# lemma-osu/sknnr

Measured on NVIDIA B200. Metric: query-neighbors/sec (kneighbors+predict, k=7), higher is better.
Workload: dtype f16 operands / f32 accumulate filter + f64 refine

## Files before the change

### sknnr_b200/csrc/search_tc.cu

```cuda
#include <cstdio>
#include "common.cuh"
#include "kernels.h"
#include "tc_common.cuh"

#include <type_traits>

namespace sk {

template <int MT_, int NS_, int CAP_, int CAPE_> struct TcCfg {
    static constexpr int MT = MT_, NS = NS_, CAP = CAP_, CAPE = CAPE_;
    static constexpr int QT = MT * TC_M;
    static constexpr int EPI_WARPS = MT * 4 * NS;
    static constexpr int THREADS = (EPI_WARPS + MT + 1) * 32;
    static constexpr int LD = QT * NS;
    static constexpr int SORT = CAP <= 16 ? 16 : 32;
    static_assert(CAP <= SORT && CAP % 2 == 0, "candidate buffer shape");
    static constexpr int CH = 4 / NS;
};

__device__ unsigned long long g_tc_counters[8];

constexpr int TC_JOINT = 10;
constexpr int TC_JOINT_WIDE = 12;


template <int KC, int CAP, int LD, int NS, int J>
__device__ __forceinline__ ThrPr tc_compact(uint32_t bs0, uint32_t pub0, uint32_t c4, float thr, uint32_t pr) {
    static_assert(KC < CAP, "the buffer needs slack above KC");
    constexpr int SORT = CAP <= 16 ? 16 : 32;
    constexpr uint32_t IOFF = CAP * LD * 4, STEP = LD * 4;
    const uint32_t cs0 = bs0 + c4;
    const int cnt = (int)(pr / STEP);
    SK_CHECK((pr & (STEP - 1)) == c4 && cnt <= CAP);
    float s[SORT];
#pragma unroll
    for (int j = 0; j < SORT; ++j) s[j] = (j < CAP && j < cnt) ? lds_f32(cs0 + j * STEP) : SK_INF_F;
    sort_regs<SORT>(s);
    float t = s[KC - 1];
    if constexpr (NS == 2 && J < 2 * KC) {
        static_assert(LD == 512, "partner column = column ^ 256");
        const uint32_t mine = pub0 + c4, other = pub0 + (c4 ^ 1024u);
        float o[KC];
#pragma unroll
        for (int i = 0; i < KC; ++i) {
            st_shared_b32(mine + i * STEP, __float_as_uint(s[i]));
            o[i] = lds_f32(other + i * STEP);
        }
        const float joint = tc_union_rank<KC, J, SORT>(s, o);
        t = fminf(t, joint);
    }
    t = fminf(t, thr);
    uint32_t w = cs0;
#pragma unroll 4
    for (int j = 0; j < CAP; ++j) {
        const float v = lds_f32(cs0 + j * STEP);
        const int id = lds_s32(cs0 + IOFF + j * STEP);
        if (j < cnt && v < t) {
            st_shared_b32(w, __float_as_uint(v));
            st_shared_b32(w + IOFF, (uint32_t)id);
            w += STEP;
        }
    }
    ThrPr out;
    out.thr = t;
    out.pr = w - bs0;
    return out;
}

template <int KC, int CAP, int LD, int CAPE, int NS, int J, bool DBG>
__device__ __noinline__ ThrPr tc_drain(uint32_t bs0, uint32_t pqv0, uint32_t pqi0, uint32_t pub0, uint32_t c4,
                                       float thr, uint32_t pr, uint32_t pqo, int dbg) {
    constexpr uint32_t IOFF = CAP * LD * 4, STEP = LD * 4, ES = LD * 32;
    constexpr uint32_t FULL = (CAP - 2) * STEP, LAST = (CAP - 1) * STEP;
    const int n_me = (int)(pqo / ES);
    SK_CHECK((pqo & (ES - 1)) == 8u * c4 && n_me <= CAPE);
    const int n_it = __reduce_max_sync(SK_FULL, n_me);
    for (int it = 0; it < n_it; ++it) {
        const bool act = it < n_me;
        if (__any_sync(SK_FULL, act && pr >= FULL)) {
            if (DBG && (dbg & 8) && (threadIdx.x & 31) == 0) atomicAdd(&g_tc_counters[4], 1ull);
            const ThrPr c = tc_compact<KC, CAP, LD, NS, J>(bs0, pub0, c4, thr, pr);
            thr = c.thr;
// ... 20 lines not shown
    out.thr = thr;
    out.pr = pr;
    out.n_it = n_it;
    return out;
}

template <int LD, int CAPE, bool DBG>
__device__ __forceinline__ void tc_chunk(const uint32_t (&r)[32], int idb, uint32_t pqv0, uint32_t pqi0, float &thr,
                                         uint32_t &pqo, int dbg) {
    constexpr uint32_t ES = LD * 32, PQ_END = CAPE * ES;
    float v[32];
#pragma unroll
    for (int i = 0; i < 32; ++i) v[i] = __uint_as_float(r[i]);
    float g[4];
#pragma unroll
    for (int o = 0; o < 4; ++o) {
        const float *w = v + 8 * o;
        g[o] = fminf(fminf(fminf(fminf(w[0], w[1]), w[2]), fminf(fminf(w[3], w[4]), w[5])), fminf(w[6], w[7]));
    }
    const float m = fminf(fminf(fminf(g[0], g[1]), g[2]), g[3]);
    const bool hit = m < thr;
    if constexpr (DBG) {
        const unsigned hits = __ballot_sync(SK_FULL, hit);
        if ((dbg & 8) && (threadIdx.x & 31) == 0) {
            atomicAdd(&g_tc_counters[0], 1ull);
            if (hits) atomicAdd(&g_tc_counters[1], 1ull);
        }
        if (hits == 0u) return;
        if (dbg & 1) return;
    } else {
        if (!__any_sync(SK_FULL, hit)) return;
    }
    unsigned ov[4];
#pragma unroll
    for (int o = 0; o < 4; ++o) ov[o] = __ballot_sync(SK_FULL, g[o] < thr);
#pragma unroll
    for (int o = 0; o < 4; ++o) {
        if (ov[o] == 0u) continue;
        const bool p = g[o] < thr;
        const bool room = pqo < PQ_END;
        SK_CHECK(pqo < PQ_END + ES);
        tc_dump8(p && room, pqv0 + pqo, pqi0 + (pqo >> 3), v + 8 * o, idb + 8 * o);
        if (p && !room) thr = fminf(thr, g[o]);
        if (p && room) pqo += ES;
        if (DBG && (dbg & 8) && p) atomicAdd(&g_tc_counters[room ? 2 : 5], 1ull);
    }
}

template <int CH, class F>
__device__ __forceinline__ void tc_epi_job(uint32_t (&R)[CH][32], uint32_t tcol, uint32_t afull_addr,
                                           uint32_t parity, uint32_t aempty_addr, int lane, F &&proc) {
    mbar_wait_addr(afull_addr, parity);
    tc_fence_after();
    if constexpr (CH == 2) {
        tmem_ld64_issue(tcol, R[0], R[1]);
    } else if constexpr (CH == 4) {
        tmem_ld64_issue(tcol, R[0], R[1]);
        tmem_ld64_issue(tcol + 64, R[2], R[3]);
    } else {
        uint32_t dep = 0;
#pragma unroll
        for (int c = 0; c < CH; ++c) tmem_ld32_issue(tcol + 32 * c, R[c], dep);
    }
#pragma unroll
    for (int c = 0; c < CH; ++c) tmem_ld_wait(R[c]);
    tc_fence_before();
    __syncwarp();
    if (lane == 0) mbar_arrive_addr(aempty_addr);
    if constexpr (CH >= 1) proc(R[0], std::integral_constant<int, 0>{});
    if constexpr (CH >= 2) proc(R[1], std::integral_constant<int, 1>{});
    if constexpr (CH >= 3) proc(R[2], std::integral_constant<int, 2>{});
    if constexpr (CH >= 4) proc(R[3], std::integral_constant<int, 3>{});
}

template <int KC, int MT, int NS, int CAP, int CAPE, int J, bool DBG>
__global__ void __launch_bounds__(TcCfg<MT, NS, CAP, CAPE>::THREADS, 1)
search_tc_kernel(const __half *__restrict__ qimg, const __half *__restrict__ rimg, int kc_tot,
                 int n_rtiles, int nstage, int n_seed, int seed_stride, long long n_q,
                 int *__restrict__ cand_idx, float *__restrict__ cand_thr, int dbg,
                 const float *__restrict__ init_thr, const int *__restrict__ n_rows_dev) {
    using Cfg = TcCfg<MT, NS, CAP, CAPE>;
    if (n_rows_dev) {
        const long long n_dev = *n_rows_dev;
        if ((long long)blockIdx.x * Cfg::QT >= n_dev) return;
        n_q = min(n_q, n_dev);
    }
    constexpr int LD = Cfg::LD, EPI_WARPS = Cfg::EPI_WARPS;
    constexpr bool JOINT = NS == 2 && J < 2 * KC;
    constexpr int KCP = JOINT ? KC : 0;
    extern __shared__ __align__(128) unsigned char smem_raw[];
    const uint32_t a_bytes = (uint32_t)kc_tot * TC_M * TC_ROWB;
    const uint32_t b_bytes = (uint32_t)kc_tot * TC_N * TC_ROWB;
    unsigned char *Qs = smem_raw;
    unsigned char *Rs = Qs + MT * a_bytes;
    float *buf_s = reinterpret_cast<float *>(Rs + (size_t)nstage * b_bytes);
    int *buf_i = reinterpret_cast<int *>(buf_s + CAP * LD);
    float *pq_v = reinterpret_cast<float *>(buf_i + CAP * LD);
    int *pq_i = reinterpret_cast<int *>(pq_v + CAPE * LD * 8);
    float *pub = reinterpret_cast<float *>(pq_i + CAPE * LD);
    uint64_t *full = reinterpret_cast<uint64_t *>(pub + KCP * LD);
    uint64_t *empty = full + nstage;
    uint64_t *afull = empty + nstage;
    uint64_t *aempty = afull + TC_SLOTS;
    uint64_t *qbar = aempty + TC_SLOTS;
    uint32_t *tmem_slot = reinterpret_cast<uint32_t *>(qbar + 1);

    const int warp = __shfl_sync(SK_FULL, (int)(threadIdx.x >> 5), 0), lane = threadIdx.x & 31;
    if (threadIdx.x == 0) {
        for (int s = 0; s < nstage; ++s) {
            mbar_init(&full[s], 1);
            mbar_init(&empty[s], MT);
        }
        for (int a = 0; a < TC_SLOTS; ++a) {
            mbar_init(&afull[a], 1);
            mbar_init(&aempty[a], 4 * NS);
        }
        mbar_init(qbar, 1);
        fence_mbar_init();
    }
    if (warp == EPI_WARPS) tmem_alloc(tmem_slot, 512);
    tc_fence_before();
    __syncthreads();
    tc_fence_after();
    const uint32_t tmem_base = *tmem_slot;
    const long long qtile = blockIdx.x;
    const int ksteps = kc_tot >> 1;
    const int n_seq = n_seed + n_rtiles;

    if (warp == EPI_WARPS + MT) {
        if (lane == 0) {
            mbar_expect_tx(qbar, MT * a_bytes);
            bulk_g2s(Qs, (const unsigned char *)qimg + (size_t)qtile * MT * a_bytes, MT * a_bytes, qbar);
            int sn = 0;
            uint32_t wrap_par = 1;
            bool wrapped = false;
            const unsigned char *rbase = (const unsigned char *)rimg;
            for (int tn = 0; tn < n_seq; ++tn) {
                if (wrapped) mbar_wait(&empty[sn], wrap_par);
                const int tile = tn < n_seed ? tn * seed_stride : tn - n_seed;
                if (DBG && (dbg & 4) && wrapped) {
                    mbar_arrive(&full[sn]);
                } else {
                    mbar_expect_tx(&full[sn], b_bytes);
                    bulk_g2s(Rs + (size_t)sn * b_bytes, rbase + (size_t)tile * b_bytes, b_bytes, &full[sn]);
                }
                if (++sn == nstage) {
                    sn = 0;
                    wrap_par = wrapped ? (wrap_par ^ 1u) : 0u;
                    wrapped = true;
                }
            }
        }
        __syncwarp();
    } else if (warp >= EPI_WARPS) {
        const int h = warp - EPI_WARPS;
        mbar_wait(qbar, 0);
        const uint32_t a_lbo = TC_M * TC_ROWB, b_lbo = TC_N * TC_ROWB;
        const uint64_t desc_hi = (uint64_t)((128u >> 4) | (1u << 14)) << 32;
        const uint32_t a_lo0 = (((smem_u32(Qs) + h * a_bytes) >> 4) & 0x3fffu) | (((a_lbo >> 4) & 0x3fffu) << 16);
        const uint32_t b_lo0 = ((smem_u32(Rs) >> 4) & 0x3fffu) | (((b_lbo >> 4) & 0x3fffu) << 16);
        const uint32_t a_kstep = (2 * a_lbo) >> 4, b_kstep = (2 * b_lbo) >> 4;
        const uint32_t b_img = b_bytes >> 4;
        int s = 0;
        uint32_t full_par = 0, b_lo_s = b_lo0;
        for (int t = 0; t < n_seq; ++t) {
            const int j = t * MT + h;
            const uint32_t sl = (uint32_t)j & (TC_SLOTS - 1);
            mbar_wait(&full[s], full_par);
            if (j >= TC_SLOTS) mbar_wait(&aempty[sl], (uint32_t)(((j >> 2) - 1) & 1));
            tc_fence_after();
            const uint32_t d_tmem = tmem_base + sl * TC_N;
            SK_CHECK(s >= 0 && s < nstage && sl < TC_SLOTS);
            if (elect_one()) {
                if (DBG && (dbg & 16)) {
                    uint32_t a2 = a_lo0, b2 = b_lo_s;
                    tc_mma_f16(d_tmem, desc_hi | a2, desc_hi | b2, TC_IDESC, 0u);
                    for (int ks = 1; ks < ksteps; ++ks) {
                        a2 += a_kstep;
                        b2 += b_kstep;
                        tc_mma_f16(d_tmem, desc_hi | a2, desc_hi | b2, TC_IDESC, 1u);
                    }
                }
                uint32_t a_lo = a_lo0, b_lo = b_lo_s;
                tc_mma_f16(d_tmem, desc_hi | a_lo, desc_hi | b_lo, TC_IDESC, 0u);
#pragma unroll 4
                for (int ks = 1; ks < ksteps; ++ks) {
                    a_lo += a_kstep;
                    b_lo += b_kstep;
                    tc_mma_f16(d_tmem, desc_hi | a_lo, desc_hi | b_lo, TC_IDESC, 1u);
                }
                tc_commit(&afull[sl]);
                tc_commit(&empty[s]);
            }
            __syncwarp();
            b_lo_s += b_img;
            if (++s == nstage) {
                s = 0;
                full_par ^= 1u;
                b_lo_s = b_lo0;
            }
        }
    } else {
        constexpr int CH = Cfg::CH;
        const int col = threadIdx.x;
        const int p = warp / (MT * 4);
        const int h = (warp >> 2) % MT;
        const int qslot = h * TC_M + (warp & 3) * 32 + lane;
        const uint32_t tlane = tmem_base + (((uint32_t)((warp & 3) * 32)) << 16) + (uint32_t)(p * CH * 32);
        float thr = SK_INF_F;
        if (init_thr) {
            const long long q_me = qtile * Cfg::QT + qslot;
            thr = q_me < n_q ? init_thr[q_me] : -SK_INF_F;
        }
        uint32_t R[CH][32];
        int t = 0;
        const uint32_t afull_a0 = smem_u32(afull), aempty_a0 = smem_u32(aempty);

        const uint32_t bs0 = smem_u32(smem_raw) + MT * a_bytes + (uint32_t)nstage * b_bytes;
        const uint32_t pqv0 = bs0 + 2u * CAP * LD * 4u, pqi0 = pqv0 + (uint32_t)CAPE * LD * 32u;
        const uint32_t pub0 = pqi0 + (uint32_t)CAPE * LD * 4u;
        const uint32_t c4 = 4u * (uint32_t)col;
        if constexpr (KCP > 0) {
#pragma unroll
            for (int i = 0; i < KCP; ++i) st_shared_b32(pub0 + c4 + i * (LD * 4), __float_as_uint(SK_INF_F));
        }

        if (n_seed > 0) {
            static_assert(2 * CAP >= TC_GROUPS, "group minima are parked in the candidate buffers");
            float *gcol = buf_s + col;
#pragma unroll
            for (int g = 0; g < TC_GROUPS; ++g) gcol[g * LD] = SK_INF_F;
            const bool fine = n_seed * CH < TC_GROUPS;
            for (; t < n_seed; ++t) {
                const int j = t * MT + h, sl = j & (TC_SLOTS - 1);
                const int g0 = (t * CH) & (TC_GROUPS - 1);
                tc_epi_job<CH>(R, tlane + (uint32_t)(sl * TC_N), afull_a0 + 8u * sl, (uint32_t)((j >> 2) & 1),
                               aempty_a0 + 8u * sl, lane,
                               [&](const uint32_t (&r)[32], auto ic) {
                                   constexpr int c = decltype(ic)::value;
                                   if (!fine) {
                                       float *g = gcol + (g0 + c) * LD;
                                       *g = fminf(*g, tc_min32(r));
                                   } else {
#pragma unroll
                                       for (int o = 0; o < 4; ++o) {
                                           float m = __uint_as_float(r[8 * o]);
#pragma unroll
                                           for (int e = 1; e < 8; ++e) m = fminf(m, __uint_as_float(r[8 * o + e]));
                                           float *g = gcol + (((t * CH + c) * 4 + o) & (TC_GROUPS - 1)) * LD;
                                           *g = fminf(*g, m);
                                       }
                                   }
                               });
            }
            float gm[TC_GROUPS];
#pragma unroll
            for (int g = 0; g < TC_GROUPS; ++g) gm[g] = gcol[g * LD];
            sort_regs<TC_GROUPS>(gm);
            thr = gm[KC - 1];
            if constexpr (KCP > 0) {
#pragma unroll
                for (int i = 0; i < KC; ++i) st_shared_b32(pub0 + c4 + i * (LD * 4), __float_as_uint(gm[i]));
                asm volatile("bar.sync %0, 64;" ::"r"(1 + (warp & (MT * 4 - 1))) : "memory");
                float o[KC];
#pragma unroll
                for (int i = 0; i < KC; ++i) o[i] = lds_f32(pub0 + (c4 ^ 1024u) + i * (LD * 4));
                const float joint = tc_union_rank<KC, J, TC_GROUPS>(gm, o);
                thr = fminf(thr, joint);
            }
        }

        constexpr uint32_t ES = LD * 32;
        uint32_t pr = c4;
        uint32_t pqo = 8u * c4;
        int since_drain = 1;
        const int early_tiles = max(64, n_rtiles >> 3);
        for (; t < n_seq; ++t) {
            const int j = t * MT + h, sl = j & (TC_SLOTS - 1);
            const int idb = (t - n_seed) * TC_N + p * CH * 32;
            tc_epi_job<CH>(R, tlane + (uint32_t)(sl * TC_N), afull_a0 + 8u * sl, (uint32_t)((j >> 2) & 1),
                           aempty_a0 + 8u * sl, lane,
                           [&](const uint32_t (&r)[32], auto ic) {
                               constexpr int c = decltype(ic)::value;
                               tc_chunk<LD, CAPE, DBG>(r, idb + c * 32, pqv0, pqi0, thr, pqo, dbg);
                           });
            constexpr int DRAIN_EVERY = 8;
            bool now;
            if constexpr (CAPE >= 4 && NS == 2) {
                now = (((t - n_seed) & (DRAIN_EVERY - 1)) == DRAIN_EVERY - 1) | (--since_drain == 0);
                if ((t - n_seed) < early_tiles) now |= __any_sync(SK_FULL, pqo >= (uint32_t)(CAPE - 1) * ES);
            } else {
                now = __any_sync(SK_FULL, pqo >= ES);
            }
            if (now) {
                if (DBG && (dbg & 8) && lane == 0) atomicAdd(&g_tc_counters[3], 1ull);
                if (DBG && (dbg & 32)) {
                    pqo = 8u * c4;
                    since_drain = -1;
                    continue;
                }
                const ThrPr d = tc_drain<KC, CAP, LD, CAPE, NS, J, DBG>(bs0, pqv0, pqi0, pub0, c4, thr, pr, pqo, dbg);
                thr = d.thr;
                pr = d.pr;
                pqo = 8u * c4;
                since_drain = d.n_it >= CAPE - 1 ? 1 : (d.n_it >= CAPE - 2 ? 2 : -1);
            }
        }

        {
            const ThrPr d = tc_drain<KC, CAP, LD, CAPE, NS, J, DBG>(bs0, pqv0, pqi0, pub0, c4, thr, pr, pqo, dbg);
            const ThrPr c = tc_compact<KC, CAP, LD, NS, J>(bs0, pub0, c4, d.thr, d.pr);
            thr = c.thr;
            pr = c.pr;
        }
        const int cnt = (int)(pr / (uint32_t)(LD * 4));
        SK_CHECK(cnt < KC && cnt <= 16 / NS);
        const long long q = qtile * Cfg::QT + qslot;
        if (q < n_q) {
            constexpr int KOUT = 16 / NS;
            int4 *dst = reinterpret_cast<int4 *>(cand_idx + (q * NS + p) * KOUT);
#pragma unroll
            for (int jj = 0; jj < KOUT; jj += 4) {
                int4 v;
                v.x = (jj + 0 < cnt) ? buf_i[(jj + 0) * LD + col] : -1;
                v.y = (jj + 1 < cnt) ? buf_i[(jj + 1) * LD + col] : -1;
                v.z = (jj + 2 < cnt) ? buf_i[(jj + 2) * LD + col] : -1;
                v.w = (jj + 3 < cnt) ? buf_i[(jj + 3) * LD + col] : -1;
                dst[jj / 4] = v;
            }
            cand_thr[q * NS + p] = thr;
        }
    }

    tc_fence_before();
    __syncthreads();
    tc_fence_after();
    if (warp == EPI_WARPS) tmem_dealloc(tmem_base, 512);
    if (DBG && (dbg & 8) && blockIdx.x == gridDim.x - 1 && threadIdx.x == 0)
        printf("tc counters (up to the last CTA): chunks %llu events %llu queued %llu drains %llu compactions %llu dropped %llu\n",
               g_tc_counters[0], g_tc_counters[1], g_tc_counters[2], g_tc_counters[3], g_tc_counters[4],
               g_tc_counters[5]);
}

int g_tc_debug = 0;

static constexpr int TC_MT = 2;

size_t search_tc_smem_bytes(int kc_tot, int nstage, int ns, int cape) {
    const size_t a = (size_t)kc_tot * TC_M * TC_ROWB, b = (size_t)kc_tot * TC_N * TC_ROWB;
    const size_t ld = (size_t)TC_MT * TC_M * ns, cap = ns == 2 ? 16 : 32, kcp = (ns == 2 && kc_tot <= 6) ? 8 : 0;
    return TC_MT * a + nstage * b + ld * 4 * (2 * cap + (size_t)cape * 9 + kcp) +
           (size_t)(2 * nstage + 2 * TC_SLOTS + 1) * 8 + 16;
}

int search_tc_pick_config(int kc_tot) {
    const int capes[2] = {4, 2};
    for (int ci = 0; ci < 2; ++ci)
        for (int s = 4; s >= 2; --s)
            if (search_tc_smem_bytes(kc_tot, s, 2, capes[ci]) <= 227 * 1024 &&
                search_tc_smem_bytes(kc_tot, s, 1, capes[ci]) <= 227 * 1024)
                return s | (capes[ci] << 8);
    return 0;
}

int search_tc_seed_stride(int n_rtiles, int seed_stride) {
    if (seed_stride <= 0) seed_stride = 4;
    if (n_rtiles < 64) return 1;
    if (n_rtiles < 192) return seed_stride < 2 ? seed_stride : 2;
    return seed_stride;
}
int search_tc_seed_tiles(int n_rtiles, int seed_stride) {
    const int st = search_tc_seed_stride(n_rtiles, seed_stride);
    return (n_rtiles + st - 1) / st;
}

template <int KC, int MT, int NS, int CAP, int CAPE, int J, bool DBG>
static cudaError_t launch_tc_dbg(const __half *qimg, const __half *rimg, int kc_tot, int n_rtiles, int nstage,
                                 int seed_stride, long long n_q, int *cand_idx, float *cand_thr,
                                 const float *init_thr, const int *n_rows_dev, cudaStream_t st) {
    using Cfg = TcCfg<MT, NS, CAP, CAPE>;
    const size_t smem = search_tc_smem_bytes(kc_tot, nstage, NS, CAPE);
    cudaError_t e = cudaFuncSetAttribute(search_tc_kernel<KC, MT, NS, CAP, CAPE, J, DBG>,
                                         cudaFuncAttributeMaxDynamicSharedMemorySize, 227 * 1024);
    if (e != cudaSuccess) return e;
    const long long n_qtiles = (n_q + Cfg::QT - 1) / Cfg::QT;
    const int n_seed = init_thr ? 0 : search_tc_seed_tiles(n_rtiles, seed_stride);
    search_tc_kernel<KC, MT, NS, CAP, CAPE, J, DBG><<<(unsigned)n_qtiles, Cfg::THREADS, smem, st>>>(
        qimg, rimg, kc_tot, n_rtiles, nstage, n_seed, search_tc_seed_stride(n_rtiles, seed_stride), n_q, cand_idx,
        cand_thr, g_tc_debug, init_thr, n_rows_dev);
    return cudaGetLastError();
}

template <int KC, int MT, int NS, int CAP>
static cudaError_t launch_tc(const __half *qimg, const __half *rimg, int kc_tot, int n_rtiles, int nstage,
                             int cape, int seed_stride, int wide_joint, long long n_q, int *cand_idx, float *cand_thr,
                             const float *init_thr, const int *n_rows_dev, cudaStream_t st) {
    constexpr int JLO = NS == 2 ? TC_JOINT : 1, JMID = NS == 2 ? TC_JOINT_WIDE : 1, JHI = NS == 2 ? 2 * KC : 1;
    const bool deep = kc_tot > 6;
#define SK_TC_GO(CAPE_, J_, DBG_)                                                                                  \
    return launch_tc_dbg<KC, MT, NS, CAP, CAPE_, J_, DBG_>(qimg, rimg, kc_tot, n_rtiles, nstage, seed_stride, n_q, \
                                                           cand_idx, cand_thr, init_thr, n_rows_dev, st)
    if (g_tc_debug && cape == 4 && !deep) SK_TC_GO(4, JLO, true);
    if (cape == 4 && !deep && NS == 2 && wide_joint) SK_TC_GO(4, JMID, false);
    if (cape == 4 && !deep) SK_TC_GO(4, JLO, false);
    if (cape == 4) SK_TC_GO(4, JHI, false);
    if (cape == 2) SK_TC_GO(2, JHI, false);
#undef SK_TC_GO
    return cudaErrorInvalidValue;
}

cudaError_t launch_search_tc(const __half *qimg, const __half *rimg, int kc_tot, int n_rtiles,
                             long long n_q, int ns, int config, int seed_stride, int wide_joint, int *cand_idx,
                             float *cand_thr, const float *init_thr, const int *n_rows_dev, cudaStream_t st) {
    if (n_q <= 0) return cudaSuccess;
    const int nstage = config & 0xff, cape = (config >> 8) & 0xff;
    if (ns == 2)
        return launch_tc<8, TC_MT, 2, 16>(qimg, rimg, kc_tot, n_rtiles, nstage, cape, seed_stride, wide_joint, n_q,
                                          cand_idx, cand_thr, init_thr, n_rows_dev, st);
    if (ns == 1)
        return launch_tc<16, TC_MT, 1, 32>(qimg, rimg, kc_tot, n_rtiles, nstage, cape, seed_stride, 0, n_q,
                                           cand_idx, cand_thr, init_thr, n_rows_dev, st);
    return cudaErrorInvalidValue;
}

}
```

### sknnr_b200/csrc/refine.cu

```cuda
#include "common.cuh"
#include "kernels.h"

namespace sk {

constexpr int REFINE_WARPS = 8;

__device__ __forceinline__ double dist2_lane(const double *__restrict__ zq, const double *__restrict__ r,
                                             int d, int h) {
    double acc = 0.0;
    for (int k = h; k < d; k += 16) {
        const double df = zq[k] - __ldg(r + k);
        acc = __fma_rn(df, df, acc);
    }
    return acc;
}
template <int DJ>
__device__ __forceinline__ double dist2_lane_regs(const double (&zr)[DJ], const double *__restrict__ r, int d,
                                                  int h) {
    double rv[DJ];
#pragma unroll
    for (int j = 0; j < DJ; ++j) rv[j] = (h + 16 * j < d) ? __ldg(r + h + 16 * j) : 0.0;
    double acc = 0.0;
#pragma unroll
    for (int j = 0; j < DJ; ++j) {
// ... 45 lines not shown
    return __double2float_ru(t);
}

template <int DJ>
__global__ void __launch_bounds__(REFINE_WARPS * 32)
refine_kernel(RefineArgs a, FinishParams fp) {
    const int warp = __shfl_sync(SK_FULL, (int)(threadIdx.x >> 5), 0), lane = threadIdx.x & 31;
    const long long q = (long long)blockIdx.x * REFINE_WARPS + warp;
    if (q >= a.n_q || (a.n_rows_dev && q >= *a.n_rows_dev)) return;
    if (a.n_rows_dev && *a.n_rows_dev < a.bypass_rows) {
        if (lane == 0) a.fb_list[atomicAdd(a.fb_count, 1)] = a.row_map ? a.row_map[q] : (int)q;
        return;
    }
    const double *zq = a.z64 + q * a.d;

    const int half = lane >> 4, hl = lane & 15;
    const bool small = a.kc <= 16;
    int id = 0x7fffffff;
    double d2 = SK_INF_D;
    const int my_c = lane < a.kc ? a.cand_idx[q * a.kc + lane] : -1;
    double zr[DJ > 0 ? DJ : 1];
    if constexpr (DJ > 0) {
#pragma unroll
        for (int j = 0; j < DJ; ++j) zr[j] = (hl + 16 * j < a.d) ? zq[hl + 16 * j] : 0.0;
    }
#pragma unroll 4
    for (int i = 0; 2 * i < a.kc; ++i) {
        const int c = __shfl_sync(SK_FULL, my_c, (2 * i + half) & 31);
        const bool have = c >= 0 && c < a.n_ref;
        double acc = 0.0;
        if (have) {
            if constexpr (DJ > 0)
                acc = dist2_lane_regs<DJ>(zr, a.ref64 + (long long)c * a.d, a.d, hl);
            else
                acc = dist2_lane(zq, a.ref64 + (long long)c * a.d, a.d, hl);
        }
        acc = dist2_reduce16(acc);
        if (small) {
            const double other = __shfl_xor_sync(SK_FULL, acc, 16);
            if ((lane >> 1) == i && lane < 16 && my_c >= 0 && my_c < a.n_ref) {
                id = my_c;
                d2 = (lane & 1) == half ? acc : other;
            }
        } else if (have && hl == (i & 15)) {
            id = c;
            d2 = acc;
        }
    }
    double qn = 0.0;
    for (int k = lane; k < a.d; k += 32) {
        const double df = zq[k] - a.mu[k];
        qn += df * df;
    }
#pragma unroll
    for (int o = 16; o > 0; o >>= 1) qn += __shfl_xor_sync(SK_FULL, qn, o);

    if (small)
        warp_sort_pairs<double, 16>(d2, id, lane);
    else
        warp_sort_pairs<double, 32>(d2, id, lane);

    const int kk = fp.k + (fp.exclude_self ? 1 : 0);
    const double kth = __shfl_sync(SK_FULL, d2, kk - 1);
    float thr = a.cand_thr[q * a.n_thr];
    for (int i = 1; i < a.n_thr; ++i) thr = fminf(thr, a.cand_thr[q * a.n_thr + i]);
    bool ok;
    if (thr == SK_INF_F) {
        ok = true;
    } else {
        const double bound = (double)thr * a.thr_scale + qn - a.eps_s * (qn + a.r2max);
        ok = kth < bound && qn < a.qn_limit;
    }
    if (!ok) {
        if (lane == 0) {
            const int pos = atomicAdd(a.fb_count, 1);
            a.fb_list[pos] = a.row_map ? a.row_map[q] : (int)q;
            if (a.fb_thr) a.fb_thr[pos] = retry_threshold(kth, qn, a);
        }
        return;
    }
    finish_query(fp, q, sqrt_padded(d2), id, lane);
}

template <int DJ>
__global__ void __launch_bounds__(REFINE_WARPS * 32)
refine2_kernel(RefineArgs a, FinishParams fp) {
    const int warp = __shfl_sync(SK_FULL, (int)(threadIdx.x >> 5), 0), lane = threadIdx.x & 31;
    const int seg = lane >> 4, hl = lane & 15;
    const long long n_rows = a.n_rows_dev ? min((long long)*a.n_rows_dev, a.n_q) : a.n_q;
    const long long q0 = ((long long)blockIdx.x * REFINE_WARPS + warp) * 2;
    if (q0 >= n_rows) return;
    const bool live = q0 + seg < n_rows;
    const long long q = live ? q0 + seg : q0;
    if (a.n_rows_dev && n_rows < a.bypass_rows) {
        if (live && hl == 0) a.fb_list[atomicAdd(a.fb_count, 1)] = a.row_map ? a.row_map[q] : (int)q;
        return;
    }
    const double *zq = a.z64 + q * a.d;
    double zr[DJ];
#pragma unroll
    for (int j = 0; j < DJ; ++j) zr[j] = (hl + 16 * j < a.d) ? zq[hl + 16 * j] : 0.0;
    const int my_c = hl < a.kc ? a.cand_idx[q * a.kc + hl] : -1;
    int id = 0x7fffffff;
    double d2 = SK_INF_D;
    auto take = [&](int i) {
        const int c = __shfl_sync(SK_FULL, my_c, i, 16);
        SK_CHECK(c >= -1 && c < a.n_ref);
        const bool have = c >= 0 && c < a.n_ref;
        double acc = 0.0;
        if (have) acc = dist2_lane_regs<DJ>(zr, a.ref64 + (long long)c * a.d, a.d, hl);
        acc = dist2_reduce16(acc);
        if (have && hl == i) {
            id = c;
            d2 = acc;
        }
    };
    const unsigned vm = __ballot_sync(SK_FULL, my_c >= 0);
    int n_step = 8;
    if (a.kc == 16) {
        int worst = 0;
        bool prefix = true;
#pragma unroll
        for (int hlf = 0; hlf < 4; ++hlf) {
            const unsigned m = (vm >> (8 * hlf)) & 0xffu;
            const int n = __popc(m);
            prefix = prefix && (m == ((1u << n) - 1u));
            worst = max(worst, n);
        }
        if (prefix) n_step = worst;
        for (int i = 0; i < n_step; ++i) {
            take(i);
            take(8 + i);
        }
    } else {
#pragma unroll 4
        for (int i = 0; i < a.kc; ++i) take(i);
    }
    double qn = 0.0;
    for (int k = hl; k < a.d; k += 16) {
        const double df = zq[k] - a.mu[k];
        qn += df * df;
    }
#pragma unroll
    for (int o = 8; o > 0; o >>= 1) qn += __shfl_xor_sync(SK_FULL, qn, o);
    warp_sort_pairs<double, 16>(d2, id, hl);

    const int kk = fp.k + (fp.exclude_self ? 1 : 0);
    const double kth = __shfl_sync(SK_FULL, d2, kk - 1, 16);
    float thr = a.cand_thr[q * a.n_thr];
    for (int i = 1; i < a.n_thr; ++i) thr = fminf(thr, a.cand_thr[q * a.n_thr + i]);
    bool ok = true;
    if (thr != SK_INF_F) ok = kth < (double)thr * a.thr_scale + qn - a.eps_s * (qn + a.r2max) && qn < a.qn_limit;
    if (live && !ok && hl == 0) {
        const int pos = atomicAdd(a.fb_count, 1);
        a.fb_list[pos] = a.row_map ? a.row_map[q] : (int)q;
        if (a.fb_thr) a.fb_thr[pos] = retry_threshold(kth, qn, a);
    }
    finish_query_w<16>(fp, q, sqrt_padded(d2), id, hl, live && ok);
}

cudaError_t launch_refine(const RefineArgs &a, const FinishParams &fp, cudaStream_t st) {
    if (a.n_q <= 0) return cudaSuccess;
    if (a.kc <= 16 && a.d <= 64) {
        const long long grid2 = (a.n_q + 2 * REFINE_WARPS - 1) / (2 * REFINE_WARPS);
        switch ((a.d + 15) / 16) {
            case 1: refine2_kernel<1><<<(unsigned)grid2, REFINE_WARPS * 32, 0, st>>>(a, fp); break;
            case 2: refine2_kernel<2><<<(unsigned)grid2, REFINE_WARPS * 32, 0, st>>>(a, fp); break;
            case 3: refine2_kernel<3><<<(unsigned)grid2, REFINE_WARPS * 32, 0, st>>>(a, fp); break;
            default: refine2_kernel<4><<<(unsigned)grid2, REFINE_WARPS * 32, 0, st>>>(a, fp); break;
        }
        return cudaGetLastError();
    }
    const long long grid = (a.n_q + REFINE_WARPS - 1) / REFINE_WARPS;
    switch (a.d <= 64 ? (a.d + 15) / 16 : 0) {
        case 1: refine_kernel<1><<<(unsigned)grid, REFINE_WARPS * 32, 0, st>>>(a, fp); break;
        case 2: refine_kernel<2><<<(unsigned)grid, REFINE_WARPS * 32, 0, st>>>(a, fp); break;
        case 3: refine_kernel<3><<<(unsigned)grid, REFINE_WARPS * 32, 0, st>>>(a, fp); break;
        case 4: refine_kernel<4><<<(unsigned)grid, REFINE_WARPS * 32, 0, st>>>(a, fp); break;
        default: refine_kernel<0><<<(unsigned)grid, REFINE_WARPS * 32, 0, st>>>(a, fp); break;
    }
    return cudaGetLastError();
}

constexpr int EXACT_THREADS = 256;

__device__ __forceinline__ double exact_pair(const ExactArgs &a, long long q, int j) {
    if (a.metric == 0) {
        const double *zq = a.z64 + q * a.d;
        const double *r = a.ref64 + (long long)j * a.d;
        return dist2_serial(zq, r, a.d);
    }
    const uint16_t *qc = a.qcodes + q * a.ldq;
    const uint16_t *rc = a.rcodes + (long long)j * a.n_trees;
    double num = 0.0;
    for (int t = 0; t < a.n_trees; ++t) {
        if (qc[t] != rc[t]) num = __dadd_rn(num, a.w[t]);
    }
    return num / a.wsum;
}

__device__ void finish_query_block(const FinishParams &p, long long q, double *sd, int *si, double *key,
                                   long long *sec, int kk) {
    __shared__ double sh_denom;
    __shared__ int sh_zero;
    const long long row = p.row_offset + q;
    if (threadIdx.x == 0) {
        if (p.exclude_self) {
            int pos = 0;
            for (int c = 0; c < kk; ++c)
                if ((long long)si[c] == row) { pos = c; break; }
            for (int c = pos; c + 1 < kk; ++c) {
                sd[c] = sd[c + 1];
                si[c] = si[c + 1];
            }
        }
        if (p.deterministic) {
            const double scale = fmax(sd[p.k - 1], 1.0);
            for (int c = 0; c < p.k; ++c) {
                key[c] = rint((sd[c] / scale) * p.round_scale) / p.round_scale;
                long long diff = (long long)si[c] - row;
                if (diff < 0) diff = -diff;
                sec[c] = (diff << 31) | (long long)si[c];
            }
            for (int c = 1; c < p.k; ++c) {
// ... 181 lines not shown
```

Before: 120.6 million.

## Make tensor-core search kernel persistent over query tiles with Q-tile reuse barrier

Turns the search kernel into a grid-stride persistent kernel capped at four blocks per SM. Each block loops over query tiles and reuses its barriers, TMEM slots and stage ring across tiles, with a new qfree barrier guarding reloads of the query image. The next query tile is also prefetched into L2. This removes per-block launch, setup and TMEM allocation costs and lets the reference stream continue across tiles. In exchange it adds cross-tile barrier parity bookkeeping and a serial dependence on the Q buffer, and the kernel declares one block per SM, so the 4x grid only runs as extra waves.

After: 120.4 million (median of 6 runs). No clear change (-0.2%).

```diff
diff --git a/sknnr_b200/csrc/search_tc.cu b/sknnr_b200/csrc/search_tc.cu
--- a/sknnr_b200/csrc/search_tc.cu
+++ b/sknnr_b200/csrc/search_tc.cu
@@ -1,3 +1,4 @@
+#include <algorithm>
 #include <cstdio>
 #include "common.cuh"
 #include "kernels.h"
@@ -184,9 +185,10 @@
     using Cfg = TcCfg<MT, NS, CAP, CAPE>;
     if (n_rows_dev) {
         const long long n_dev = *n_rows_dev;
-        if ((long long)blockIdx.x * Cfg::QT >= n_dev) return;
         n_q = min(n_q, n_dev);
     }
+    const long long n_qtiles = (n_q + Cfg::QT - 1) / Cfg::QT;
+    if ((long long)blockIdx.x >= n_qtiles) return;
     constexpr int LD = Cfg::LD, EPI_WARPS = Cfg::EPI_WARPS;
     constexpr bool JOINT = NS == 2 && J < 2 * KC;
     constexpr int KCP = JOINT ? KC : 0;
@@ -205,7 +207,8 @@
     uint64_t *afull = empty + nstage;
     uint64_t *aempty = afull + TC_SLOTS;
     uint64_t *qbar = aempty + TC_SLOTS;
-    uint32_t *tmem_slot = reinterpret_cast<uint32_t *>(qbar + 1);
+    uint64_t *qfree = qbar + 1;
+    uint32_t *tmem_slot = reinterpret_cast<uint32_t *>(qfree + 1);
 
     const int warp = __shfl_sync(SK_FULL, (int)(threadIdx.x >> 5), 0), lane = threadIdx.x & 31;
     if (threadIdx.x == 0) {
@@ -218,6 +221,7 @@
             mbar_init(&aempty[a], 4 * NS);
         }
         mbar_init(qbar, 1);
+        mbar_init(qfree, MT);
         fence_mbar_init();
     }
     if (warp == EPI_WARPS) tmem_alloc(tmem_slot, 512);
@@ -225,38 +229,45 @@
     __syncthreads();
     tc_fence_after();
     const uint32_t tmem_base = *tmem_slot;
-    const long long qtile = blockIdx.x;
     const int ksteps = kc_tot >> 1;
-    const int n_seq = n_seed + n_rtiles;
+    const int n_seq = (DBG && (dbg & 64)) ? n_seed : n_seed + n_rtiles;
 
     if (warp == EPI_WARPS + MT) {
         if (lane == 0) {
-            mbar_expect_tx(qbar, MT * a_bytes);
-            bulk_g2s(Qs, (const unsigned char *)qimg + (size_t)qtile * MT * a_bytes, MT * a_bytes, qbar);
             int sn = 0;
             uint32_t wrap_par = 1;
             bool wrapped = false;
-            const unsigned char *rbase = (const unsigned char *)rimg;
-            for (int tn = 0; tn < n_seq; ++tn) {
-                if (wrapped) mbar_wait(&empty[sn], wrap_par);
-                const int tile = tn < n_seed ? tn * seed_stride : tn - n_seed;
-                if (DBG && (dbg & 4) && wrapped) {
-                    mbar_arrive(&full[sn]);
-                } else {
-                    mbar_expect_tx(&full[sn], b_bytes);
-                    bulk_g2s(Rs + (size_t)sn * b_bytes, rbase + (size_t)tile * b_bytes, b_bytes, &full[sn]);
-                }
-                if (++sn == nstage) {
-                    sn = 0;
-                    wrap_par = wrapped ? (wrap_par ^ 1u) : 0u;
-                    wrapped = true;
+            const unsigned char *rbase = (const unsigned char *)rimg, *qbase = (const unsigned char *)qimg;
+            int it = 0;
+            for (long long qtile = blockIdx.x; qtile < n_qtiles; qtile += gridDim.x, ++it) {
+                if (it > 0) mbar_wait(qfree, (uint32_t)((it - 1) & 1));
+                mbar_expect_tx(qbar, MT * a_bytes);
+                bulk_g2s(Qs, qbase + (size_t)qtile * MT * a_bytes, MT * a_bytes, qbar);
+                if (qtile + gridDim.x < n_qtiles)
+                    asm volatile("cp.async.bulk.prefetch.L2.global [%0], %1;" ::"l"(
+                                     qbase + (size_t)(qtile + gridDim.x) * MT * a_bytes),
+                                 "r"(MT * a_bytes)
+                                 : "memory");
+                for (int tn = 0; tn < n_seq; ++tn) {
+                    if (wrapped) mbar_wait(&empty[sn], wrap_par);
+                    const int tile = tn < n_seed ? tn * seed_stride : tn - n_seed;
+                    if (DBG && (dbg & 4) && wrapped) {
+                        mbar_arrive(&full[sn]);
+                    } else {
+                        mbar_expect_tx(&full[sn], b_bytes);
+                        bulk_g2s(Rs + (size_t)sn * b_bytes, rbase + (size_t)tile * b_bytes, b_bytes, &full[sn]);
+                    }
+                    if (++sn == nstage) {
+                        sn = 0;
+                        wrap_par = wrapped ? (wrap_par ^ 1u) : 0u;
+                        wrapped = true;
+                    }
                 }
             }
         }
         __syncwarp();
     } else if (warp >= EPI_WARPS) {
         const int h = warp - EPI_WARPS;
-        mbar_wait(qbar, 0);
         const uint32_t a_lbo = TC_M * TC_ROWB, b_lbo = TC_N * TC_ROWB;
         const uint64_t desc_hi = (uint64_t)((128u >> 4) | (1u << 14)) << 32;
         const uint32_t a_lo0 = (((smem_u32(Qs) + h * a_bytes) >> 4) & 0x3fffu) | (((a_lbo >> 4) & 0x3fffu) << 16);
@@ -265,42 +276,49 @@
         const uint32_t b_img = b_bytes >> 4;
         int s = 0;
         uint32_t full_par = 0, b_lo_s = b_lo0;
-        for (int t = 0; t < n_seq; ++t) {
-            const int j = t * MT + h;
-            const uint32_t sl = (uint32_t)j & (TC_SLOTS - 1);
-            mbar_wait(&full[s], full_par);
-            if (j >= TC_SLOTS) mbar_wait(&aempty[sl], (uint32_t)(((j >> 2) - 1) & 1));
-            tc_fence_after();
-            const uint32_t d_tmem = tmem_base + sl * TC_N;
-            SK_CHECK(s >= 0 && s < nstage && sl < TC_SLOTS);
-            if (elect_one()) {
-                if (DBG && (dbg & 16)) {
-                    uint32_t a2 = a_lo0, b2 = b_lo_s;
-                    tc_mma_f16(d_tmem, desc_hi | a2, desc_hi | b2, TC_IDESC, 0u);
+        int it = 0;
+        for (long long qtile = blockIdx.x; qtile < n_qtiles; qtile += gridDim.x, ++it) {
+            mbar_wait(qbar, (uint32_t)(it & 1));
+            const int jb = it * n_seq * MT;
+            for (int t = 0; t < n_seq; ++t) {
+                const int j = jb + t * MT + h;
+                const uint32_t sl = (uint32_t)j & (TC_SLOTS - 1);
+                mbar_wait(&full[s], full_par);
+                if (j >= TC_SLOTS) mbar_wait(&aempty[sl], (uint32_t)(((j >> 2) - 1) & 1));
+                tc_fence_after();
+                const uint32_t d_tmem = tmem_base + sl * TC_N;
+                SK_CHECK(s >= 0 && s < nstage && sl < TC_SLOTS);
+                if (elect_one()) {
+                    if (DBG && (dbg & 16)) {
+                        uint32_t a2 = a_lo0, b2 = b_lo_s;
+                        tc_mma_f16(d_tmem, desc_hi | a2, desc_hi | b2, TC_IDESC, 0u);
+                        for (int ks = 1; ks < ksteps; ++ks) {
+                            a2 += a_kstep;
+                            b2 += b_kstep;
+                            tc_mma_f16(d_tmem, desc_hi | a2, desc_hi | b2, TC_IDESC, 1u);
+                        }
+                    }
+                    uint32_t a_lo = a_lo0, b_lo = b_lo_s;
+                    tc_mma_f16(d_tmem, desc_hi | a_lo, desc_hi | b_lo, TC_IDESC, 0u);
+#pragma unroll 4
                     for (int ks = 1; ks < ksteps; ++ks) {
-                        a2 += a_kstep;
-                        b2 += b_kstep;
-                        tc_mma_f16(d_tmem, desc_hi | a2, desc_hi | b2, TC_IDESC, 1u);
+                        a_lo += a_kstep;
+                        b_lo += b_kstep;
+                        tc_mma_f16(d_tmem, desc_hi | a_lo, desc_hi | b_lo, TC_IDESC, 1u);
                     }
-                }
-                uint32_t a_lo = a_lo0, b_lo = b_lo_s;
-                tc_mma_f16(d_tmem, desc_hi | a_lo, desc_hi | b_lo, TC_IDESC, 0u);
-#pragma unroll 4
-                for (int ks = 1; ks < ksteps; ++ks) {
-                    a_lo += a_kstep;
-                    b_lo += b_kstep;
-                    tc_mma_f16(d_tmem, desc_hi | a_lo, desc_hi | b_lo, TC_IDESC, 1u);
-                }
-                tc_commit(&afull[sl]);
-                tc_commit(&empty[s]);
-            }
+                    tc_commit(&afull[sl]);
+                    tc_commit(&empty[s]);
+                }
+                __syncwarp();
+                b_lo_s += b_img;
+                if (++s == nstage) {
+                    s = 0;
+                    full_par ^= 1u;
+                    b_lo_s = b_lo0;
+                }
+            }
+            if (elect_one()) tc_commit(qfree);
             __syncwarp();
-            b_lo_s += b_img;
-            if (++s == nstage) {
-                s = 0;
-                full_par ^= 1u;
-                b_lo_s = b_lo0;
-            }
         }
     } else {
         constexpr int CH = Cfg::CH;
@@ -309,128 +327,132 @@
         const int h = (warp >> 2) % MT;
         const int qslot = h * TC_M + (warp & 3) * 32 + lane;
         const uint32_t tlane = tmem_base + (((uint32_t)((warp & 3) * 32)) << 16) + (uint32_t)(p * CH * 32);
-        float thr = SK_INF_F;
-        if (init_thr) {
-            const long long q_me = qtile * Cfg::QT + qslot;
-            thr = q_me < n_q ? init_thr[q_me] : -SK_INF_F;
-        }
-        uint32_t R[CH][32];
-        int t = 0;
-        const uint32_t afull_a0 = smem_u32(afull), aempty_a0 = smem_u32(aempty);
-
-        const uint32_t bs0 = smem_u32(smem_raw) + MT * a_bytes + (uint32_t)nstage * b_bytes;
-        const uint32_t pqv0 = bs0 + 2u * CAP * LD * 4u, pqi0 = pqv0 + (uint32_t)CAPE * LD * 32u;
-        const uint32_t pub0 = pqi0 + (uint32_t)CAPE * LD * 4u;
-        const uint32_t c4 = 4u * (uint32_t)col;
-        if constexpr (KCP > 0) {
-#pragma unroll
-            for (int i = 0; i < KCP; ++i) st_shared_b32(pub0 + c4 + i * (LD * 4), __float_as_uint(SK_INF_F));
-        }
-
-        if (n_seed > 0) {
-            static_assert(2 * CAP >= TC_GROUPS, "group minima are parked in the candidate buffers");
-            float *gcol = buf_s + col;
-#pragma unroll
-            for (int g = 0; g < TC_GROUPS; ++g) gcol[g * LD] = SK_INF_F;
-            const bool fine = n_seed * CH < TC_GROUPS;
-            for (; t < n_seed; ++t) {
-                const int j = t * MT + h, sl = j & (TC_SLOTS - 1);
-                const int g0 = (t * CH) & (TC_GROUPS - 1);
+        int it = 0;
+        for (long long qtile = blockIdx.x; qtile < n_qtiles; qtile += gridDim.x, ++it) {
+            const int jb = it * n_seq * MT;
+            float thr = SK_INF_F;
+            if (init_thr) {
+                const long long q_me = qtile * Cfg::QT + qslot;
+                thr = q_me < n_q ? init_thr[q_me] : -SK_INF_F;
+            }
+            uint32_t R[CH][32];
+            int t = 0;
+            const uint32_t afull_a0 = smem_u32(afull), aempty_a0 = smem_u32(aempty);
+
+            const uint32_t bs0 = smem_u32(smem_raw) + MT * a_bytes + (uint32_t)nstage * b_bytes;
+            const uint32_t pqv0 = bs0 + 2u * CAP * LD * 4u, pqi0 = pqv0 + (uint32_t)CAPE * LD * 32u;
+            const uint32_t pub0 = pqi0 + (uint32_t)CAPE * LD * 4u;
+            const uint32_t c4 = 4u * (uint32_t)col;
+            if constexpr (KCP > 0) {
+#pragma unroll
+                for (int i = 0; i < KCP; ++i) st_shared_b32(pub0 + c4 + i * (LD * 4), __float_as_uint(SK_INF_F));
+            }
+
+            if (n_seed > 0) {
+                static_assert(2 * CAP >= TC_GROUPS, "group minima are parked in the candidate buffers");
+                float *gcol = buf_s + col;
+#pragma unroll
+                for (int g = 0; g < TC_GROUPS; ++g) gcol[g * LD] = SK_INF_F;
+                const bool fine = n_seed * CH < TC_GROUPS;
+                for (; t < n_seed; ++t) {
+                    const int j = jb + t * MT + h, sl = j & (TC_SLOTS - 1);
+                    const int g0 = (t * CH) & (TC_GROUPS - 1);
+                    tc_epi_job<CH>(R, tlane + (uint32_t)(sl * TC_N), afull_a0 + 8u * sl, (uint32_t)((j >> 2) & 1),
+                                   aempty_a0 + 8u * sl, lane,
+                                   [&](const uint32_t (&r)[32], auto ic) {
+                                       constexpr int c = decltype(ic)::value;
+                                       if (!fine) {
+                                           float *g = gcol + (g0 + c) * LD;
+                                           *g = fminf(*g, tc_min32(r));
+                                       } else {
+#pragma unroll
+                                           for (int o = 0; o < 4; ++o) {
+                                               float m = __uint_as_float(r[8 * o]);
+#pragma unroll
+                                               for (int e = 1; e < 8; ++e) m = fminf(m, __uint_as_float(r[8 * o + e]));
+                                               float *g = gcol + (((t * CH + c) * 4 + o) & (TC_GROUPS - 1)) * LD;
+                                               *g = fminf(*g, m);
+                                           }
+                                       }
+                                   });
+                }
+                float gm[TC_GROUPS];
+#pragma unroll
+                for (int g = 0; g < TC_GROUPS; ++g) gm[g] = gcol[g * LD];
+                sort_regs<TC_GROUPS>(gm);
+                thr = gm[KC - 1];
+                if constexpr (KCP > 0) {
+#pragma unroll
+                    for (int i = 0; i < KC; ++i) st_shared_b32(pub0 + c4 + i * (LD * 4), __float_as_uint(gm[i]));
+                    asm volatile("bar.sync %0, 64;" ::"r"(1 + (warp & (MT * 4 - 1))) : "memory");
+                    float o[KC];
+#pragma unroll
+                    for (int i = 0; i < KC; ++i) o[i] = lds_f32(pub0 + (c4 ^ 1024u) + i * (LD * 4));
+                    const float joint = tc_union_rank<KC, J, TC_GROUPS>(gm, o);
+                    thr = fminf(thr, joint);
+                }
+            }
+
+            constexpr uint32_t ES = LD * 32;
+            uint32_t pr = c4;
+            uint32_t pqo = 8u * c4;
+            int since_drain = 1;
+            const int early_tiles = max(64, n_rtiles >> 3);
+            for (; t < n_seq; ++t) {
+                const int j = jb + t * MT + h, sl = j & (TC_SLOTS - 1);
+                const int idb = (t - n_seed) * TC_N + p * CH * 32;
                 tc_epi_job<CH>(R, tlane + (uint32_t)(sl * TC_N), afull_a0 + 8u * sl, (uint32_t)((j >> 2) & 1),
                                aempty_a0 + 8u * sl, lane,
                                [&](const uint32_t (&r)[32], auto ic) {
                                    constexpr int c = decltype(ic)::value;
-                                   if (!fine) {
-                                       float *g = gcol + (g0 + c) * LD;
-                                       *g = fminf(*g, tc_min32(r));
-                                   } else {
-#pragma unroll
-                                       for (int o = 0; o < 4; ++o) {
-                                           float m = __uint_as_float(r[8 * o]);
-#pragma unroll
-                                           for (int e = 1; e < 8; ++e) m = fminf(m, __uint_as_float(r[8 * o + e]));
-                                           float *g = gcol + (((t * CH + c) * 4 + o) & (TC_GROUPS - 1)) * LD;
-                                           *g = fminf(*g, m);
-                                       }
-                                   }
+                                   tc_chunk<LD, CAPE, DBG>(r, idb + c * 32, pqv0, pqi0, thr, pqo, dbg);
                                });
-            }
-            float gm[TC_GROUPS];
-#pragma unroll
-            for (int g = 0; g < TC_GROUPS; ++g) gm[g] = gcol[g * LD];
-            sort_regs<TC_GROUPS>(gm);
-            thr = gm[KC - 1];
-            if constexpr (KCP > 0) {
-#pragma unroll
-                for (int i = 0; i < KC; ++i) st_shared_b32(pub0 + c4 + i * (LD * 4), __float_as_uint(gm[i]));
-                asm volatile("bar.sync %0, 64;" ::"r"(1 + (warp & (MT * 4 - 1))) : "memory");
-                float o[KC];
-#pragma unroll
-                for (int i = 0; i < KC; ++i) o[i] = lds_f32(pub0 + (c4 ^ 1024u) + i * (LD * 4));
-                const float joint = tc_union_rank<KC, J, TC_GROUPS>(gm, o);
-                thr = fminf(thr, joint);
-            }
-        }
-
-        constexpr uint32_t ES = LD * 32;
-        uint32_t pr = c4;
-        uint32_t pqo = 8u * c4;
-        int since_drain = 1;
-        const int early_tiles = max(64, n_rtiles >> 3);
-        for (; t < n_seq; ++t) {
-            const int j = t * MT + h, sl = j & (TC_SLOTS - 1);
-            const int idb = (t - n_seed) * TC_N + p * CH * 32;
-            tc_epi_job<CH>(R, tlane + (uint32_t)(sl * TC_N), afull_a0 + 8u * sl, (uint32_t)((j >> 2) & 1),
-                           aempty_a0 + 8u * sl, lane,
-                           [&](const uint32_t (&r)[32], auto ic) {
-                               constexpr int c = decltype(ic)::value;
-                               tc_chunk<LD, CAPE, DBG>(r, idb + c * 32, pqv0, pqi0, thr, pqo, dbg);
-                           });
-            constexpr int DRAIN_EVERY = 8;
-            bool now;
-            if constexpr (CAPE >= 4 && NS == 2) {
-                now = (((t - n_seed) & (DRAIN_EVERY - 1)) == DRAIN_EVERY - 1) | (--since_drain == 0);
-                if ((t - n_seed) < early_tiles) now |= __any_sync(SK_FULL, pqo >= (uint32_t)(CAPE - 1) * ES);
-            } else {
-                now = __any_sync(SK_FULL, pqo >= ES);
-            }
-            if (now) {
-                if (DBG && (dbg & 8) && lane == 0) atomicAdd(&g_tc_counters[3], 1ull);
-                if (DBG && (dbg & 32)) {
+                constexpr int DRAIN_EVERY = 8;
+                bool now;
+                if constexpr (CAPE >= 4 && NS == 2) {
+                    now = (((t - n_seed) & (DRAIN_EVERY - 1)) == DRAIN_EVERY - 1) | (--since_drain == 0);
+                    if ((t - n_seed) < early_tiles) now |= __any_sync(SK_FULL, pqo >= (uint32_t)(CAPE - 1) * ES);
+                } else {
+                    now = __any_sync(SK_FULL, pqo >= ES);
+                }
+                if (now) {
+                    if (DBG && (dbg & 8) && lane == 0) atomicAdd(&g_tc_counters[3], 1ull);
+                    if (DBG && (dbg & 32)) {
+                        pqo = 8u * c4;
+                        since_drain = -1;
+                        continue;
+                    }
+                    const ThrPr d = tc_drain<KC, CAP, LD, CAPE, NS, J, DBG>(bs0, pqv0, pqi0, pub0, c4, thr, pr, pqo, dbg);
+                    thr = d.thr;
+                    pr = d.pr;
                     pqo = 8u * c4;
-                    since_drain = -1;
-                    continue;
-                }
+                    since_drain = d.n_it >= CAPE - 1 ? 1 : (d.n_it >= CAPE - 2 ? 2 : -1);
+                }
+            }
+
+            {
                 const ThrPr d = tc_drain<KC, CAP, LD, CAPE, NS, J, DBG>(bs0, pqv0, pqi0, pub0, c4, thr, pr, pqo, dbg);
-                thr = d.thr;
-                pr = d.pr;
-                pqo = 8u * c4;
-                since_drain = d.n_it >= CAPE - 1 ? 1 : (d.n_it >= CAPE - 2 ? 2 : -1);
-            }
-        }
-
-        {
-            const ThrPr d = tc_drain<KC, CAP, LD, CAPE, NS, J, DBG>(bs0, pqv0, pqi0, pub0, c4, thr, pr, pqo, dbg);
-            const ThrPr c = tc_compact<KC, CAP, LD, NS, J>(bs0, pub0, c4, d.thr, d.pr);
-            thr = c.thr;
-            pr = c.pr;
-        }
-        const int cnt = (int)(pr / (uint32_t)(LD * 4));
-        SK_CHECK(cnt < KC && cnt <= 16 / NS);
-        const long long q = qtile * Cfg::QT + qslot;
-        if (q < n_q) {
-            constexpr int KOUT = 16 / NS;
-            int4 *dst = reinterpret_cast<int4 *>(cand_idx + (q * NS + p) * KOUT);
-#pragma unroll
-            for (int jj = 0; jj < KOUT; jj += 4) {
-                int4 v;
-                v.x = (jj + 0 < cnt) ? buf_i[(jj + 0) * LD + col] : -1;
-                v.y = (jj + 1 < cnt) ? buf_i[(jj + 1) * LD + col] : -1;
-                v.z = (jj + 2 < cnt) ? buf_i[(jj + 2) * LD + col] : -1;
-                v.w = (jj + 3 < cnt) ? buf_i[(jj + 3) * LD + col] : -1;
-                dst[jj / 4] = v;
-            }
-            cand_thr[q * NS + p] = thr;
+                const ThrPr c = tc_compact<KC, CAP, LD, NS, J>(bs0, pub0, c4, d.thr, d.pr);
+                thr = c.thr;
+                pr = c.pr;
+            }
+            const int cnt = (int)(pr / (uint32_t)(LD * 4));
+            SK_CHECK(cnt < KC && cnt <= 16 / NS);
+            const long long q = qtile * Cfg::QT + qslot;
+            if (q < n_q) {
+                constexpr int KOUT = 16 / NS;
+                int4 *dst = reinterpret_cast<int4 *>(cand_idx + (q * NS + p) * KOUT);
+#pragma unroll
+                for (int jj = 0; jj < KOUT; jj += 4) {
+                    int4 v;
+                    v.x = (jj + 0 < cnt) ? buf_i[(jj + 0) * LD + col] : -1;
+                    v.y = (jj + 1 < cnt) ? buf_i[(jj + 1) * LD + col] : -1;
+                    v.z = (jj + 2 < cnt) ? buf_i[(jj + 2) * LD + col] : -1;
+                    v.w = (jj + 3 < cnt) ? buf_i[(jj + 3) * LD + col] : -1;
+                    dst[jj / 4] = v;
+                }
+                cand_thr[q * NS + p] = thr;
+            }
         }
     }
 
@@ -452,7 +474,7 @@
     const size_t a = (size_t)kc_tot * TC_M * TC_ROWB, b = (size_t)kc_tot * TC_N * TC_ROWB;
     const size_t ld = (size_t)TC_MT * TC_M * ns, cap = ns == 2 ? 16 : 32, kcp = (ns == 2 && kc_tot <= 6) ? 8 : 0;
     return TC_MT * a + nstage * b + ld * 4 * (2 * cap + (size_t)cape * 9 + kcp) +
-           (size_t)(2 * nstage + 2 * TC_SLOTS + 1) * 8 + 16;
+           (size_t)(2 * nstage + 2 * TC_SLOTS + 2) * 8 + 16;
 }
 
 int search_tc_pick_config(int kc_tot) {
@@ -485,9 +507,12 @@
     cudaError_t e = cudaFuncSetAttribute(search_tc_kernel<KC, MT, NS, CAP, CAPE, J, DBG>,
                                          cudaFuncAttributeMaxDynamicSharedMemorySize, 227 * 1024);
     if (e != cudaSuccess) return e;
+    int dev = 0, n_sm = 148;
+    if (cudaGetDevice(&dev) == cudaSuccess) cudaDeviceGetAttribute(&n_sm, cudaDevAttrMultiProcessorCount, dev);
     const long long n_qtiles = (n_q + Cfg::QT - 1) / Cfg::QT;
+    const long long grid = std::min<long long>(n_qtiles, 4LL * n_sm);
     const int n_seed = init_thr ? 0 : search_tc_seed_tiles(n_rtiles, seed_stride);
-    search_tc_kernel<KC, MT, NS, CAP, CAPE, J, DBG><<<(unsigned)n_qtiles, Cfg::THREADS, smem, st>>>(
+    search_tc_kernel<KC, MT, NS, CAP, CAPE, J, DBG><<<(unsigned)grid, Cfg::THREADS, smem, st>>>(
         qimg, rimg, kc_tot, n_rtiles, nstage, n_seed, search_tc_seed_stride(n_rtiles, seed_stride), n_q, cand_idx,
         cand_thr, g_tc_debug, init_thr, n_rows_dev);
     return cudaGetLastError();
```

## Batch refine distance reductions with transpose-style butterfly across candidates

Applied to the files above, without the earlier changes.

Replaces the per-candidate 16-lane shuffle reduction in the refine kernel with a batched scheme. Each lane computes partial distances for up to 16 candidates, paired across half-groups, then performs a recursive-halving transpose reduction so every lane ends up holding its own candidate's full distance. This cuts the number of shuffles per candidate and removes the per-candidate select. It also adds a minBlocks launch bound for small DJ and computes the query norm from registers instead of global memory. The trade-off is higher register pressure from the 8-element partial array. It also changes the fallback path for kc<16, which now loops only min(kc,8) times, paired.

Result: faster. 121.6 million before, 123.4 million after (median of 6 runs) (+1.5%).

```diff
diff --git a/sknnr_b200/csrc/refine.cu b/sknnr_b200/csrc/refine.cu
--- a/sknnr_b200/csrc/refine.cu
+++ b/sknnr_b200/csrc/refine.cu
@@ -151,8 +151,19 @@
     finish_query(fp, q, sqrt_padded(d2), id, lane);
 }
 
+template <int N>
+__device__ __forceinline__ void reduce_half(double (&v)[2 * N], int m, int hl) {
+    const bool up = (hl & m) != 0;
+#pragma unroll
+    for (int k = 0; k < N; ++k) {
+        const double keep = up ? v[k + N] : v[k];
+        const double send = up ? v[k] : v[k + N];
+        v[k] = keep + __shfl_xor_sync(SK_FULL, send, m);
+    }
+}
+
 template <int DJ>
-__global__ void __launch_bounds__(REFINE_WARPS * 32)
+__global__ void __launch_bounds__(REFINE_WARPS * 32, DJ <= 2 ? 6 : 1)
 refine2_kernel(RefineArgs a, FinishParams fp) {
     const int warp = __shfl_sync(SK_FULL, (int)(threadIdx.x >> 5), 0), lane = threadIdx.x & 31;
     const int seg = lane >> 4, hl = lane & 15;
@@ -170,22 +181,9 @@
 #pragma unroll
     for (int j = 0; j < DJ; ++j) zr[j] = (hl + 16 * j < a.d) ? zq[hl + 16 * j] : 0.0;
     const int my_c = hl < a.kc ? a.cand_idx[q * a.kc + hl] : -1;
-    int id = 0x7fffffff;
-    double d2 = SK_INF_D;
-    auto take = [&](int i) {
-        const int c = __shfl_sync(SK_FULL, my_c, i, 16);
-        SK_CHECK(c >= -1 && c < a.n_ref);
-        const bool have = c >= 0 && c < a.n_ref;
-        double acc = 0.0;
-        if (have) acc = dist2_lane_regs<DJ>(zr, a.ref64 + (long long)c * a.d, a.d, hl);
-        acc = dist2_reduce16(acc);
-        if (have && hl == i) {
-            id = c;
-            d2 = acc;
-        }
-    };
+    SK_CHECK(my_c >= -1 && my_c < a.n_ref);
     const unsigned vm = __ballot_sync(SK_FULL, my_c >= 0);
-    int n_step = 8;
+    int n_step = min(a.kc, 8);
     if (a.kc == 16) {
         int worst = 0;
         bool prefix = true;
@@ -197,18 +195,36 @@
             worst = max(worst, n);
         }
         if (prefix) n_step = worst;
-        for (int i = 0; i < n_step; ++i) {
-            take(i);
-            take(8 + i);
-        }
-    } else {
-#pragma unroll 4
-        for (int i = 0; i < a.kc; ++i) take(i);
-    }
+    }
+    const int hi = hl & 8;
+    double pa[8];
+#pragma unroll
+    for (int i = 0; i < 8; ++i) {
+        pa[i] = 0.0;
+        if (i < n_step) {
+            const int ca = __shfl_sync(SK_FULL, my_c, i + hi, 16);
+            const int cb = __shfl_sync(SK_FULL, my_c, i + 8 - hi, 16);
+            const bool ha = ca >= 0 && ca < a.n_ref, hb = cb >= 0 && cb < a.n_ref;
+            const double pb = dist2_lane_regs<DJ>(zr, a.ref64 + (size_t)(unsigned)(hb ? cb : 0) * (unsigned)a.d,
+                                                  hb ? a.d : 0, hl);
+            pa[i] = dist2_lane_regs<DJ>(zr, a.ref64 + (size_t)(unsigned)(ha ? ca : 0) * (unsigned)a.d, ha ? a.d : 0, hl);
+            pa[i] += __shfl_xor_sync(SK_FULL, pb, 8);
+        }
+    }
+    reduce_half<4>(pa, 4, hl);
+    reduce_half<2>(*reinterpret_cast<double(*)[4]>(pa), 2, hl);
+    reduce_half<1>(*reinterpret_cast<double(*)[2]>(pa), 1, hl);
+    const bool have = my_c >= 0 && my_c < a.n_ref;
+    int id = have ? my_c : 0x7fffffff;
+    double d2 = have ? pa[0] : SK_INF_D;
+
     double qn = 0.0;
-    for (int k = hl; k < a.d; k += 16) {
-        const double df = zq[k] - a.mu[k];
-        qn += df * df;
+#pragma unroll
+    for (int j = 0; j < DJ; ++j) {
+        if (hl + 16 * j < a.d) {
+            const double df = zr[j] - a.mu[hl + 16 * j];
+            qn = __fma_rn(df, df, qn);
+        }
     }
 #pragma unroll
     for (int o = 8; o > 0; o >>= 1) qn += __shfl_xor_sync(SK_FULL, qn, o);
```
